# andreistana05/SAT-MPI-Stana-Andrei

Hardware: AMD Instinct MI355X
Metric: instances solved/sec, random 3-SAT n=100 α=4.26; unit-props/sec; HBM GB/s (higher is better)
Workload: dtype int32

## Files before the change

sat-mpi-stana-andrei_amd/csrc/dpll_scan.hip:

```cpp
#include <hip/hip_runtime.h>

#include <algorithm>
#include <climits>
#include <type_traits>

#include "common.h"
#include "dpll_scan.h"

#ifndef SATMI_SCAN_WAVES_PER_SIMD
#define SATMI_SCAN_WAVES_PER_SIMD 8
#endif

namespace satmi {
namespace {

#ifdef SATMI_PHASE_STAMPS
struct PhaseClock {
    uint64_t acc[8];
    uint64_t cnt[16];
    uint64_t t;
    __device__ void start() {
        for (int i = 0; i < 8; ++i) acc[i] = 0;
        for (int i = 0; i < 16; ++i) cnt[i] = 0;
        t = __builtin_amdgcn_s_memtime();
    }
    __device__ void count(int i, uint64_t v = 1) { cnt[i] += v; }
    __device__ void mark(int i) {
        const uint64_t x = __builtin_amdgcn_s_memtime();
        acc[i] += x - t;
        t = x;
    }
};
#else
struct PhaseClock {
    __device__ void start() {}
    __device__ void mark(int) {}
    __device__ void count(int, uint64_t = 1) {}
};
#endif
enum { PH_STAGE = 0, PH_ASSIGN = 1, PH_UNITS = 2, PH_CONFLICT = 3, PH_COUNTS = 4, PH_CHOOSE = 5, PH_PURE = 6,
       PH_OTHER = 7 };

constexpr uint32_t NONE32 = 0xFFFFFFFFu;


constexpr uint32_t LV_TRUE = 8u, LV_FALSE = 0u, LV_FREE = 1u;
constexpr uint32_t CODE_PAD = 0u, CODE_DUMMY = 1u;
__device__ __forceinline__ bool sum_true(uint32_t s) { return (s & 0xF8u) != 0u; }
__device__ __forceinline__ bool sum_open(uint32_t s) { return s < 8u; }
__device__ __forceinline__ uint32_t sum_nfree(uint32_t s) { return s & 7u; }

template <int K>
struct Pack;
template <>
struct Pack<3> {
    using W = uint32_t;
    static constexpr int BITS = 10;
    static constexpr int MAXV = 511;
    static constexpr int UNROLL = 7;
};
template <>
struct Pack<5> {
    using W = uint64_t;
    static constexpr int BITS = 12;
    static constexpr int MAXV = 2047;
    static constexpr int UNROLL = 2;
};

__host__ __device__ __forceinline__ int padded_clauses(int m) { return (m + 63) & ~63; }

template <int K>
__device__ __forceinline__ uint32_t field(typename Pack<K>::W w, int j) {
    return (uint32_t)(w >> (Pack<K>::BITS * j)) & ((1u << Pack<K>::BITS) - 1u);
}

struct ScanLayout {
    uint32_t cls, lv, ts, cnt, first, trail, fvar, ftrail, scratch, occ_off, bm, bytes;
    int32_t mcap, ncap, nw;
};

struct ScanArgs {
    const int32_t *inst_clause_begin, *clause_lit_begin, *lits, *inst_nvars;
    int32_t num_instances, sol_cap, sol_stride;
    int64_t max_solutions, node_limit;
    uint64_t time_limit_ticks;
    int32_t *status;
    int64_t *counters;
    int32_t *sol_len, *sol_lits, *root_len, *root_lits;
    uint32_t *work_counter;
    uint16_t *occ;
    int32_t occ_cap;
    ScanLayout lay;
    struct SplitCfg *split;
    int32_t occ_lists;
    uint32_t snap_lds;
};

template <int K, typename C>
struct SLds {
    static constexpr uint32_t PHASE_BIT = 1u << (8 * sizeof(C) - 1);
    typename Pack<K>::W *cls;
    uint8_t *lv;
    uint32_t *ts;
    uint32_t *cnt;
    uint32_t *first;
    C *trail;
    C *fvar;
    C *ftrail;
    C *snap;
    uint32_t *plist;
    C *snapg;
    uint32_t scap;
    uint16_t *occ_off;
    uint2 *bm;
    const uint16_t *occ;
};

__device__ __forceinline__ void lv_assign(uint8_t *lv, uint32_t code) {
    lv[code] = (uint8_t)LV_TRUE;
    lv[code ^ 1u] = (uint8_t)LV_FALSE;
}
__device__ __forceinline__ void lv_clear(uint8_t *lv, uint32_t v) {
    *(uint16_t *)(lv + 2 * v) = (uint16_t)(LV_FREE | (LV_FREE << 8));
}
__device__ __forceinline__ bool var_free(const uint8_t *lv, uint32_t v) { return (lv[2 * v] & 1u) != 0u; }

#include "dpll_scan_access.h"

template <int K, typename C>
constexpr bool plist_vars() { return sizeof(C) == 2 && K == 3; }
template <int K, typename C>
constexpr bool cnt_packed() {
#ifdef SATMI_CNT_PACK_ALL
    return K == 3;
#else
    return sizeof(C) == 2 && K == 3;
#endif
}
template <int K, typename C>
__device__ __forceinline__ void cnt_inc(const SLds<K, C> &S, uint32_t code, uint32_t inc) {
    if constexpr (!cnt_packed<K, C>()) atomicAdd(&S.cnt[code], inc);
    else atomicAdd(&S.cnt[code >> 1], inc << ((code & 1u) << 4));
}
template <int K, typename C>
__device__ __forceinline__ uint32_t cnt_fetch_inc(const SLds<K, C> &S, uint32_t code) {
    if constexpr (!cnt_packed<K, C>()) {
        return atomicAdd(&S.cnt[code], 1u);
    } else {
        const uint32_t sh = (code & 1u) << 4;
        return (atomicAdd(&S.cnt[code >> 1], 1u << sh) >> sh) & 0xFFFFu;
    }
}
template <int K, typename C>
__device__ __forceinline__ uint32_t cnt_get(const SLds<K, C> &S, uint32_t code) {
    if constexpr (!cnt_packed<K, C>()) return S.cnt[code];
    else return (S.cnt[code >> 1] >> ((code & 1u) << 4)) & 0xFFFFu;
}
template <int K, typename C>
__device__ __forceinline__ uint2 cnt_pair(const SLds<K, C> &S, uint32_t v) {
    if constexpr (!cnt_packed<K, C>()) {
        return ((const uint2 *)S.cnt)[v];
    } else {
        const uint32_t w = S.cnt[v];
        return make_uint2(w & 0xFFFFu, w >> 16);
    }
}
template <int K, typename C>
__device__ __forceinline__ void cnt_clear_var(const SLds<K, C> &S, uint32_t v) {
    if constexpr (!cnt_packed<K, C>()) ((uint2 *)S.cnt)[v] = make_uint2(0u, 0u);
    else S.cnt[v] = 0u;
}


template <int K, int U, typename C, typename F>
__device__ __forceinline__ void chunk_group(const SLds<K, C> &S, int c0, F &&f) {
    using W = typename Pack<K>::W;
// ... 21 lines not shown
    for (; c0 < mpad; c0 += 64) {
        const W w = S.cls[c0 + ln];
        uint32_t x[K];
#pragma unroll
        for (int j = 0; j < K; ++j) x[j] = lv_get(S, field<K>(w, j));
        f(c0 + ln, w, x);
    }
}

template <int K>
__device__ __forceinline__ uint32_t clause_sum(const uint32_t (&x)[K]) {
    uint32_t s = x[0];
#pragma unroll
    for (int j = 1; j < K; ++j) s += x[j];
    return s;
}

template <int K>
__device__ __forceinline__ uint32_t unit_code(typename Pack<K>::W w, const uint32_t (&x)[K]) {
    if constexpr (K == 3) {
        return __builtin_amdgcn_ubfe((uint32_t)w, x[1] * (uint32_t)Pack<3>::BITS + x[2] * (2u * Pack<3>::BITS),
                                     Pack<3>::BITS);
    } else {
        uint32_t code = field<K>(w, 0);
#pragma unroll
        for (int j = 1; j < K; ++j)
            if (x[j] & 1u) code = field<K>(w, j);
        return code;
    }
}

constexpr uint32_t EPOCH_LIMIT = 0xFFFFu - 4096u;
__device__ __forceinline__ uint32_t stamp(uint32_t ep, uint32_t k) { return ((ep << 16) | 0xFFFFu) - k; }
__device__ __forceinline__ uint32_t stamp_index(uint32_t st) { return 0xFFFFu - (st & 0xFFFFu); }

template <int K, typename C>
__device__ __forceinline__ void snap_put(const SLds<K, C> &S, uint32_t k, uint32_t code) {
    if constexpr (sizeof(C) == 1) {
        S.snap[k] = (C)code;
    } else {
        if (k < S.scap) S.snap[k] = (C)code;
        else S.snapg[k - S.scap] = (C)code;
    }
}
template <int K, typename C>
__device__ __forceinline__ uint32_t snap_get(const SLds<K, C> &S, uint32_t k) {
    if constexpr (sizeof(C) == 1) return S.snap[k];
    else return k < S.scap ? (uint32_t)S.snap[k] : (uint32_t)S.snapg[k - S.scap];
}
template <int K, typename C>
__device__ __forceinline__ void snap_ready(const SLds<K, C> &S, int nu) {
    if constexpr (sizeof(C) == 2)
        if ((uint32_t)nu > S.scap) __builtin_amdgcn_fence(__ATOMIC_SEQ_CST, "workgroup");
}

template <int K, typename C>
__device__ int scan_units(const SLds<K, C> &S, int mpad, uint32_t ep, uint32_t bep, int *empty_at) {
    using W = typename Pack<K>::W;
    const uint64_t lt = lanemask_lt();
    int nu = 0;
    int e = INT_MAX;
    for_chunks<K, Pack<K>::UNROLL>(S, mpad, [&](int c, W, const uint32_t(&x)[K]) {
        const uint32_t s = clause_sum<K>(x);
        const bool open = !sum_true(s);
        const uint32_t nf = sum_nfree(s);
        if (open && nf == 0u) {
            const W w = S.cls[c];
            int t = -1;
#pragma unroll
            for (int j = 0; j < K; ++j) {
                const uint32_t code = field<K>(w, j);
                const uint32_t st = code > CODE_DUMMY ? S.ts[code >> 1] : 0u;
                if ((st >> 16) == bep) t = max(t, (int)stamp_index(st));
            }
            e = min(e, t);
        }
        const bool unit = open && nf == 1u;
        const uint64_t mk = __ballot(unit);
        if (unit) {
            const uint32_t k = (uint32_t)nu + (uint32_t)__popcll(mk & lt);
            const uint32_t code = unit_code<K>(S.cls[c], x);
            snap_put(S, k, code);
            ts_stamp(S, code >> 1, stamp(ep, k));
        }
        nu += __popcll(mk);
    });
    wave_sync();
    *empty_at = __ballot(e != INT_MAX) ? wave_min_i32(e) : INT_MAX;
    return nu;
}

template <int K, typename C>
__device__ __forceinline__ int emptier(const SLds<K, C> &S, typename Pack<K>::W w, uint32_t bep) {
    int tt = -1;
#pragma unroll
    for (int j = 0; j < K; ++j) {
        const uint32_t code = field<K>(w, j);
        const uint32_t ts = S.ts[code >> 1];
        const uint32_t st = code > CODE_DUMMY ? ts : 0u;
        tt = (st >> 16) == bep ? max(tt, (int)stamp_index(st)) : tt;
    }
    return tt;
}

constexpr int FAST_UNITS = 2;
constexpr int FAST_BATCH = 16;

template <int K, typename C>
__device__ int inc_units(const SLds<K, C> &S, int nw, int rs, int tl, uint32_t ep, uint32_t bep, int *empty_at,
                         int *pre, PhaseClock &ph) {
    using W = typename Pack<K>::W;
    const int ln = lane_id();
    ph.count(0);
    ph.count(7, (uint64_t)(tl - rs));
    if (__builtin_expect(tl - rs <= FAST_BATCH, 1)) {
        const bool inb = ln < tl - rs;
        const uint32_t x = (uint32_t)S.trail[inb ? rs + ln : rs] ^ 1u;
        const int o0 = S.occ_off[x], o1 = S.occ_off[x + 1];
        const int ob = inb ? o0 : 0, len = inb ? o1 - o0 : 0;
        const int incl = row_incl_scan(len);
        const int excl = incl - len;
        const int delta = ob - excl;
        const int total = __builtin_amdgcn_readlane(incl, 15);
        if (__builtin_expect(total <= 64, 1)) {
            ph.count(1);
            int d = __builtin_amdgcn_readlane(delta, 0);
            if (tl - rs > 1)
            for (int b = 1; b < tl - rs; ++b) {
                const int eb = __builtin_amdgcn_readlane(excl, b);
                const int db = __builtin_amdgcn_readlane(delta, b);
                d = ln >= eb ? db : d;
            }
            const bool valid = ln < total;
            const uint32_t c = S.occ[(uint32_t)(valid ? d + ln : 0)];
            const W w = cls_at(S, c);
            uint32_t x[K];
#pragma unroll
            for (int j = 0; j < K; ++j) x[j] = lv_get(S, field<K>(w, j));
            const uint32_t sv = valid ? clause_sum<K>(x) : 0xFFu;
            const bool empty = sv == 0u;
            if (__builtin_expect(__ballot(empty) != 0ull, 0)) {
                ph.count(2);
                const int et = emptier<K>(S, w, bep);
                const int e = empty ? et : INT_MAX;
                *empty_at = wave_min_i32(e);
                return 0;
            }
            *empty_at = INT_MAX;
            const bool unit = sv == 1u;
            const uint64_t um = __ballot(unit);
            const int nun = __popcll(um);
            ph.count(4, (uint64_t)nun);
            ph.count(nun == 0 ? 10 : nun == 1 ? 11 : nun == 2 ? 12 : nun <= 8 ? 13 : 6, nun <= 8 ? 1 : 0);
            if (__builtin_expect(nun <= FAST_UNITS, 1)) {
                ph.count(3);
                uint64_t dm = um;
                int rank = 0;
                const uint32_t code = unit_code<K>(w, x);
                bool keep = unit;
                int nkeep = nun;
                if (nun == 2) {
                    const int u0 = __builtin_ctzll(um), u1 = 63 - __builtin_clzll(um);
                    const uint32_t c0 = (uint32_t)__builtin_amdgcn_readlane((int)c, u0);
                    const uint32_t c1 = (uint32_t)__builtin_amdgcn_readlane((int)c, u1);
                    const uint32_t v0 = (uint32_t)__builtin_amdgcn_readlane((int)code, u0) >> 1;
                    const uint32_t v1 = (uint32_t)__builtin_amdgcn_readlane((int)code, u1) >> 1;
                    dm = c0 == c1 ? 1ull << u0 : um;
                    rank = ln == u0 ? (c1 < c0 ? 1 : 0) : (c0 < c1 ? 1 : 0);
                    const bool one = (c0 == c1) | (v0 == v1);
                    keep = unit & (!one | (rank == 0));
                    nkeep = one ? 1 : 2;
                }
                if (keep) {
                    S.trail[tl + rank] = (C)code;
                    lv_assign(S.lv, code);
                    S.ts[code >> 1] = stamp(ep, (uint32_t)rank);
                }
                wave_sync();
                *pre = nkeep;
                return __popcll(dm);
            }
            if (unit) atomicOr(&S.bm[c >> 5].x, 1u << (c & 31u));
            wave_sync();
            int nu = 0;
            if (nw <= 64) {
                const uint32_t bits = ln < nw ? S.bm[ln].x : 0u;
                const int pc = __popc(bits);
                const int in = wave_incl_scan(pc);
                if (ln < nw) S.bm[ln].y = (uint32_t)(in - pc);
                nu = lane63(in);
            } else
            for (int w0 = 0; w0 < nw; w0 += 64) {
                const int wi = w0 + ln;
                const uint32_t bits = wi < nw ? S.bm[wi].x : 0u;
                const int pc = __popc(bits);
                const int in = wave_incl_scan(pc);
                if (wi < nw) S.bm[wi].y = (uint32_t)(nu + in - pc);
                nu += lane63(in);
            }
            wave_sync();
            if (unit) {
                const uint2 pb = S.bm[c >> 5];
                const uint32_t k = pb.y + (uint32_t)__popc(pb.x & ((1u << (c & 31u)) - 1u));
                const uint32_t code = unit_code<K>(w, x);
                snap_put(S, k, code);
                ts_stamp(S, code >> 1, stamp(ep, k));
                S.bm[c >> 5].x = 0u;
            }
            wave_sync();
            ph.count(6);
            return nu;
        }
    }
    ph.count(5);
    ph.count(tl - rs > FAST_BATCH ? 8 : 9);
    int e = INT_MAX;
    int passes = 0;
    bool unit = false;
    uint32_t uc = 0, ucode = 0;
    for (int i0 = rs; i0 < tl; i0 += 64) {
        const int i = i0 + ln;
        int ob = 0, len = 0;
        if (i < tl) {
            const uint32_t x = (uint32_t)S.trail[i] ^ 1u;
            ob = S.occ_off[x];
            len = (int)S.occ_off[x + 1] - ob;
        }
        const int incl = wave_incl_scan(len);
        const int excl = incl - len;
        const int delta = ob - excl;
        const int total = lane63(incl);
        const int nb = min(64, tl - i0);
        for (int t0 = 0; t0 < total; t0 += 64) {
            const int t = t0 + ln;
            int d = 0;
            for (int b = 0; b < nb; ++b) {
                const int eb = __builtin_amdgcn_readlane(excl, b);
                const int db = __builtin_amdgcn_readlane(delta, b);
                d = t >= eb ? db : d;
            }
            ++passes;
            if (t < total) {
                const uint32_t c = S.occ[d + t];
                const W w = cls_at(S, c);
                uint32_t x[K];
#pragma unroll
                for (int j = 0; j < K; ++j) x[j] = lv_get(S, field<K>(w, j));
                const uint32_t s = clause_sum<K>(x);
                if (!sum_true(s)) {
                    const uint32_t nf = sum_nfree(s);
                    if (nf == 0u) {
                        e = min(e, emptier<K>(S, w, bep));
                    } else if (nf == 1u) {
                        atomicOr(&S.bm[c >> 5].x, 1u << (c & 31u));
                        unit = true;
                        uc = c;
                        ucode = unit_code<K>(w, x);
                    }
                }
            }
        }
    }
    wave_sync();
    const int emp = __ballot(e != INT_MAX) ? wave_min_i32(e) : INT_MAX;
    *empty_at = emp;
    if (emp != INT_MAX) {
        for (int w = ln; w < nw; w += 64) S.bm[w].x = 0u;
        wave_sync();
        return 0;
    }
    int nu = 0;
    for (int w0 = 0; w0 < nw; w0 += 64) {
        const int w = w0 + ln;
        const uint32_t bits = w < nw ? S.bm[w].x : 0u;
        const int pc = __popc(bits);
        const int in = wave_incl_scan(pc);
        if (w < nw) S.bm[w].y = (uint32_t)(nu + in - pc);
        nu += lane63(in);
    }
    wave_sync();
    if (passes <= 1) {
        if (unit) {
            const uint2 p = S.bm[uc >> 5];
            const uint32_t k = p.y + (uint32_t)__popc(p.x & ((1u << (uc & 31u)) - 1u));
            snap_put(S, k, ucode);
            ts_stamp(S, ucode >> 1, stamp(ep, k));
        }
    } else {
        for (int w = ln; w < nw; w += 64) {
            const uint2 p = S.bm[w];
            uint32_t bits = p.x, k = p.y;
            while (bits) {
                const uint32_t c = ((uint32_t)w << 5) | (uint32_t)__builtin_ctz(bits);
                bits &= bits - 1u;
                const W wd = S.cls[c];
                uint32_t x[K];
#pragma unroll
                for (int j = 0; j < K; ++j) x[j] = lv_get(S, field<K>(wd, j));
                const uint32_t code = unit_code<K>(wd, x);
                snap_put(S, k, code);
                ts_stamp(S, code >> 1, stamp(ep, k));
                ++k;
            }
        }
    }
    wave_sync();
    for (int w = ln; w < nw; w += 64) S.bm[w].x = 0u;
    return nu;
}

template <int K, typename C>
__device__ uint32_t next_decision_epoch(const SLds<K, C> &S, int n, uint32_t ep) {
    if (ep < EPOCH_LIMIT) return ep + 1;
    for (int v = lane_id(); v <= n; v += 64) S.ts[v] = 0u;
    wave_sync();
    return 1;
}

template <int K, typename C>
__device__ __forceinline__ void assign_decision(const SLds<K, C> &S, int tl, uint32_t code, uint32_t ep) {
    S.trail[tl] = (C)code;
    lv_assign(S.lv, code);
    S.ts[code >> 1] = stamp(ep, 0u);
}

template <int K, bool INC, typename C>
__device__ bool propagate(const SLds<K, C> &S, int mpad, int &tl, int nu, bool dec, uint32_t &ep, uint32_t &props,
                          uint32_t &rounds, PhaseClock &ph) {
    const int ln = lane_id();
    int e = INT_MAX;
    int rs = tl;
    props -= dec ? 1u : 0u;
    ph.count(14);
// ... 133 lines not shown
    int npure = 0;
    uint32_t lmax = 0;
    auto count_step = [&](int v0) {
        const int v = v0 + ln;
        const uint32_t vc = (uint32_t)min(v, n);
        const bool live = (v <= n) & var_free(S.lv, vc);
        const uint2 c = cnt_pair(S, vc);
        const uint32_t p = c.x, q = c.y;
        lmax = live ? max(lmax, p + q) : lmax;
        npure += __popcll(__ballot(live & ((p + q) != 0u) & ((p == 0u) | (q == 0u))));
    };
    if constexpr (sizeof(C) == 1) {
        if (n >= 1) count_step(1);
        if (n >= 65) count_step(65);
    } else {
        for (int v0 = 1; v0 <= n; v0 += 64) count_step(v0);
    }
    const uint32_t maxc = wave_max_u32(lmax);
    int ncand = 0;
    uint32_t cvar = 0;
    auto flag_step = [&](int v0) {
        const int v = v0 + ln;
        const uint32_t vc = (uint32_t)min(v, n);
        const bool live = (v <= n) & var_free(S.lv, vc);
        const uint2 c = cnt_pair(S, vc);
        const uint32_t p = c.x, q = c.y;
        const bool pure = live & ((p + q) != 0u) & ((p == 0u) | (q == 0u));
        const bool cand = live & (p + q == maxc);
        const uint64_t cm = __ballot(cand);
        cvar = (ncand == 0 && cm) ? (uint32_t)v0 + (uint32_t)__builtin_ctzll(cm) : cvar;
        ncand += __popcll(cm);
        const uint32_t vw = v <= n ? vc : 0u;
        S.first[vw] = npure ? (pure ? NONE32 : 0u) : (cand ? 1u : 0u);
        cnt_clear_var(S, vw);
    };
    if constexpr (sizeof(C) == 1) {
        if (n >= 1) flag_step(1);
        if (n >= 65) flag_step(65);
    } else {
        for (int v0 = 1; v0 <= n; v0 += 64) flag_step(v0);
    }
    cnt_clear_var(S, 0u);
    S.first[0] = 0u;
    wave_sync();
    uint32_t best = 0;
    if (npure > 0) {
        first_of_pures<K>(S, mpad, npure);
        int k = 0;
        auto collect = [&](int v0) {
            const int v = v0 + ln;
            const uint32_t f = v <= n ? S.first[v] : 0u;
            const bool pure = f != 0u;
            const uint64_t mk = __ballot(pure);
            if constexpr (!plist_vars<K, C>()) {
                if (pure) S.plist[k + __popcll(mk & lt)] = f - 1u;
            } else {
                if (pure) ((C *)S.plist)[k + __popcll(mk & lt)] = (C)v;
            }
            k += __popcll(mk);
        };
        if constexpr (sizeof(C) == 1) {
            if (n >= 1) collect(1);
            if (n >= 65) collect(65);
        } else {
            for (int v0 = 1; v0 <= n; v0 += 64) collect(v0);
        }
        wave_sync();
    } else if (maxc > 0) {
        if (ncand == 1) {
            best = cvar;
        } else {
            const uint32_t bestf = first_flagged<K>(S, mpad);
            best = uniform_u32(field<K>(S.cls[bestf >> 3], (int)(bestf & 7u)) >> 1);
        }
    }
    return {npure, best};
}

template <int K, typename C>
__device__ int assign_pures(const SLds<K, C> &S, int npure, int tl) {
    const int ln = lane_id();
    const auto pos = [&](int j) -> uint32_t {
        if constexpr (!plist_vars<K, C>()) return S.plist[j];
        else return S.first[((const C *)S.plist)[j]] - 1u;
    };
    for (int i0 = 0; i0 < npure; i0 += 64) {
        const int i = i0 + ln;
        const uint32_t my = i < npure ? pos(i) : NONE32;
        int rank = 0;
        for (int j = 0; j < npure; ++j) rank += pos(j) < my ? 1 : 0;
        if (i < npure) {
            const uint32_t code = field<K>(S.cls[my >> 3], (int)(my & 7u));
            S.trail[tl + rank] = (C)code;
            lv_assign(S.lv, code);
        }
    }
    wave_sync();
    return tl + npure;
}

template <int K, typename C>
__device__ void store_assignment(const SLds<K, C> &S, int tl, int32_t *out) {
    for (int i = lane_id(); i < tl; i += 64) {
        const uint32_t code = S.trail[i];
        const int v = (int)(code >> 1);
        out[i] = (code & 1u) ? -v : v;
    }
}

enum { ST_PROPAGATE = 0, ST_ANALYZE = 1, ST_BACKTRACK = 2, ST_DONE = 3 };

template <int K, typename C>
__device__ void build_occurrences(const SLds<K, C> &S, uint16_t *occ, int m, int n) {
    using W = typename Pack<K>::W;
    const int ln = lane_id();
    auto each_slot = [&](auto &&f) {
        for (int c = ln; c < m; c += 64) {
            const W w = S.cls[c];
#pragma unroll
            for (int j = 0; j < K; ++j) {
                const uint32_t code = field<K>(w, j);
                bool dup = code <= CODE_DUMMY;
#pragma unroll
                for (int i = 0; i < j; ++i) dup |= field<K>(w, i) == code;
                if (!dup) f(c, code);
            }
        }
    };
    each_slot([&](int, uint32_t code) { cnt_inc(S, code, 1u); });
    wave_sync();
    int carry = 0;
    for (int x0 = 0; x0 < 2 * (n + 1); x0 += 64) {
        const int x = x0 + ln;
        const int cx = x < 2 * (n + 1) ? (int)cnt_get(S, (uint32_t)x) : 0;
        const int in = wave_incl_scan(cx);
        if (x < 2 * (n + 1)) {
            S.occ_off[x] = (uint16_t)(carry + in - cx);
            if constexpr (!cnt_packed<K, C>()) S.cnt[x] = 0u;
            else if (!(x & 1)) S.cnt[x >> 1] = 0u;
        }
        carry += lane63(in);
    }
    if (ln == 0) S.occ_off[2 * (n + 1)] = (uint16_t)carry;
    wave_sync();
    each_slot([&](int c, uint32_t code) {
        const uint32_t old = cnt_fetch_inc(S, code);
        occ[S.occ_off[code] + old] = (uint16_t)c;
    });
    wave_sync();
    if constexpr (!cnt_packed<K, C>())
        for (int x = ln; x < 2 * (n + 1); x += 64) S.cnt[x] = 0u;
    else
        for (int v = ln; v <= n; v += 64) S.cnt[v] = 0u;
    __builtin_amdgcn_fence(__ATOMIC_SEQ_CST, "workgroup");
    wave_sync();
}

struct Ctr32 {
    uint32_t nodes = 0, decisions = 0, props = 0, pures = 0, conflicts = 0, rounds = 0;
};
constexpr uint32_t FLUSH_NODES = 1u << 20;
constexpr uint32_t TIME_CHECK_NODES = 1024;

#define SATMI_RLX_AGENT __ATOMIC_RELAXED, __HIP_MEMORY_SCOPE_AGENT
template <typename T>
__device__ __forceinline__ T ld_agent(T *p) { return __hip_atomic_load(p, SATMI_RLX_AGENT); }
template <typename T>
__device__ __forceinline__ void st_agent(T *p, T v) { __hip_atomic_store(p, v, SATMI_RLX_AGENT); }
template <typename T>
__device__ __forceinline__ T add_agent(T *p, T v) { return __hip_atomic_fetch_add(p, v, SATMI_RLX_AGENT); }
template <typename T>
__device__ __forceinline__ T cas_agent(T *p, T expect, T v) {
    __hip_atomic_compare_exchange_strong(p, &expect, v, __ATOMIC_RELAXED, __ATOMIC_RELAXED, __HIP_MEMORY_SCOPE_AGENT);
    return expect;
}

__device__ uint64_t flush_counters(int64_t *ctr, Ctr32 &c, bool &flushed) {
    uint64_t total = 0;
    if (lane_id() == 0) {
        const uint32_t v[6] = {c.nodes, c.decisions, c.props, c.pures, c.conflicts, c.rounds};
        const int k[6] = {SATMI_CTR_NODES, SATMI_CTR_DECISIONS, SATMI_CTR_UNIT_PROPS, SATMI_CTR_PURE,
                          SATMI_CTR_CONFLICTS, SATMI_CTR_ROUNDS};
        if (!flushed) {
            for (int i = 0; i < 6; ++i) st_agent(&ctr[k[i]], (int64_t)v[i]);
            total = c.nodes;
        } else {
            total = (uint64_t)add_agent(&ctr[SATMI_CTR_NODES], (int64_t)c.nodes) + c.nodes;
            for (int i = 1; i < 6; ++i) add_agent(&ctr[k[i]], (int64_t)v[i]);
        }
    }
    flushed = true;
    c = Ctr32{};
    return (uint64_t)uniform_u32((uint32_t)total) | ((uint64_t)uniform_u32((uint32_t)(total >> 32)) << 32);
}

struct SplitCfg {
    uint32_t pub;
    uint32_t taken;
    uint32_t pad0[30];
    int32_t want;
    uint32_t pad1[31];
    uint32_t done;
    int32_t helpers;
    uint32_t claims, reclaims;
    unsigned long long handoffs;
    unsigned long long busy;
    uint32_t pad2[24];
    int32_t slot_cap, slot_bytes, dstack_cap;
    uint32_t epoch;
    int32_t max_helpers;
    uint32_t warm;
    int32_t cont_off;
    int32_t cont_fb;
    uint32_t pad3[24];
};
constexpr int SPLIT_POOL_OFF = 512;
static_assert(sizeof(SplitCfg) == SPLIT_POOL_OFF, "SplitCfg layout");
#ifndef SATMI_SPLIT_CHECK_NODES
#define SATMI_SPLIT_CHECK_NODES 64u
#endif
constexpr uint32_t SPLIT_CHECK_NODES = SATMI_SPLIT_CHECK_NODES;
constexpr int SPLIT_MAX_PER_WAVE = 8;
enum : uint32_t { SL_PENDING = 1, SL_RUNNING = 2, SL_DONE = 3, SL_RECLAIMED = 4, SL_HANDED = 5 };
struct SlotFlags {
    uint32_t state;
    uint32_t cancel;
};
struct SlotHdr {
    int32_t inst, tl0, dec_code, status, model_len;
    int32_t cont_task, cont_depth, cont_nd;
    int64_t ctr[SATMI_NCOUNTERS];
};
constexpr int SLOT_HDR_OFF = 128, SLOT_TRAIL_OFF = 256;
__host__ __device__ __forceinline__ int slot_frames_bytes(int ncap, int cb) { return ((ncap + 1) * cb + 127) & ~127; }
__host__ __device__ __forceinline__ int slot_cont_off(int ncap, int cb) {
    return SLOT_TRAIL_OFF + slot_frames_bytes(ncap, cb);
}
__host__ __device__ __forceinline__ int slot_bytes_for(int ncap, int cb) {
    return slot_cont_off(ncap, cb) + 2 * slot_frames_bytes(ncap, cb) + ((4 * (ncap + 1) + 127) & ~127);
}

struct SlotRef {
    SlotFlags *f;
    SlotHdr *h;
    uint32_t *trail;
};
__device__ __forceinline__ SlotRef slot_ref(const ScanArgs &A, int s) {
    unsigned char *p = (unsigned char *)A.split + SPLIT_POOL_OFF + (size_t)s * (size_t)A.split->slot_bytes;
    return {(SlotFlags *)p, (SlotHdr *)(p + SLOT_HDR_OFF), (uint32_t *)(p + SLOT_TRAIL_OFF)};
}
__device__ __forceinline__ uint32_t slot_state(const ScanArgs &A, uint32_t st) { return A.split->epoch << 4 | st; }
__device__ __forceinline__ int32_t *split_dstack(const SplitCfg *cfg, size_t w) {
    unsigned char *p = (unsigned char *)cfg + SPLIT_POOL_OFF + (size_t)cfg->slot_cap * (size_t)cfg->slot_bytes;
    return (int32_t *)p + w * (size_t)cfg->dstack_cap;
}

__device__ __forceinline__ void publish_state(uint32_t *flag, uint32_t v) {
    asm volatile("s_waitcnt vmcnt(0)" ::: "memory");
    if (lane_id() == 0) st_agent(flag, v);
}
__device__ __forceinline__ void acquire_agent() {
    __builtin_amdgcn_fence(__ATOMIC_ACQUIRE, "agent");
    asm volatile("s_waitcnt vmcnt(0)" ::: "memory");
}

__device__ __forceinline__ void put_words(uint32_t *dst, const void *lds, int nbytes) {
    const uint32_t *src = (const uint32_t *)lds;
    for (int i = lane_id_here(); 4 * i < nbytes; i += 64) st_agent(&dst[i], src[i]);
}

__device__ uint32_t next_event_after(const ScanArgs &A, uint64_t total) {
    uint64_t ev = A.time_limit_ticks ? TIME_CHECK_NODES : FLUSH_NODES;
    if (A.node_limit > 0) ev = min(ev, (uint64_t)A.node_limit + 1u - total);
    return (uint32_t)ev;
}

template <int K, typename C>
__device__ void try_donate(const ScanArgs &A, const SLds<K, C> &S, int depth, int b, int32_t *dst, int &nd) {
    constexpr uint32_t PHASE = SLds<K, C>::PHASE_BIT, DON = SLds<K, C>::PHASE_BIT;
    const int ln = lane_id_here();
    int old = 0;
    if (ln == 0) old = add_agent(&A.split->want, -1);
    if (uniform_i32(old) <= 0) {
        if (ln == 0) add_agent(&A.split->want, 1);
        return;
    }
    int j = -1;
    for (int d0 = 0; d0 < depth; d0 += 64) {
        const int d = d0 + ln;
        const bool open = d < depth && !((uint32_t)S.fvar[d] & PHASE) && !((uint32_t)S.ftrail[d] & DON);
        const uint64_t mk = __ballot(open);
        if (mk) {
            j = d0 + __builtin_ctzll(mk);
            break;
        }
    }
    int s = -1;
    if (j >= 0 && nd < A.split->dstack_cap) {
        uint32_t x = 0;
        if (ln == 0) x = add_agent(&A.split->pub, 1u);
        x = uniform_u32(x);
        if (x < (uint32_t)A.split->slot_cap) s = (int)x;
    }
    if (s < 0) {
        if (ln == 0) add_agent(&A.split->want, 1);
        return;
// ... 218 lines not shown
            bool leaf = false;
            Choice r{0, 0u};
            ph.mark(PH_OTHER);
            const int nact = scan_counts<K>(S, mpad);
            ph.mark(PH_COUNTS);
            if (nact == 0) {
                leaf = true;
            } else {
                r = choose<K>(S, n, mpad);
                if (r.npure == 0 && r.best_var == 0u) leaf = true;
            }
            ph.mark(PH_CHOOSE);
            if (!leaf && r.npure > 0) {
                tl = assign_pures<K>(S, r.npure, tl);
                ph.mark(PH_PURE);
                c.pures += (uint32_t)r.npure;
                ++c.nodes;
            } else if (!leaf) {
                const uint32_t v = r.best_var;
                ep = next_decision_epoch<K>(S, n, ep);
                if (ln == 0) {
                    S.fvar[depth] = (C)v;
                    S.ftrail[depth] = (C)tl;
                    assign_decision<K>(S, tl, v << 1, ep);
                }
                ++depth;
                ++c.decisions;
                ++c.nodes;
                nu = 1;
                dec_round = true;
                state = ST_PROPAGATE;
                wave_sync();
            } else {
                if (is_task) {
                    const SlotRef me = slot_ref(A, task);
                    put_words(me.trail, S.trail, tl * (int)sizeof(C));
                    if (lane_id_here() == 0) st_agent(&me.h->model_len, tl);
                } else if (sols < A.sol_cap) {
                    store_assignment<K>(S, tl, A.sol_lits + ((int64_t)b * A.sol_cap + sols) * A.sol_stride);
                    if (ln == 0) A.sol_len[(int64_t)b * A.sol_cap + sols] = tl;
                }
                ++sols;
                if (A.max_solutions > 0 && sols >= A.max_solutions) {
                    status = SATMI_DPLL_STOPPED;
                    state = ST_DONE;
                } else {
                    state = ST_BACKTRACK;
                }
            }
        }
        if (!SPLIT && state == ST_BACKTRACK) {
            state = ST_DONE;
            int top = depth - 1;
            while (top >= 0 && (uniform_u32(S.fvar[top]) & SLds<K, C>::PHASE_BIT)) --top;
            depth = top + 1;
            if (top >= 0) {
                const uint32_t fv = uniform_u32(S.fvar[top]);
                const int ft = (int)uniform_u32(S.ftrail[top]);
                for (int i = ft + lane_id_here(); i < tl; i += 64) lv_clear(S.lv, S.trail[i] >> 1);
                tl = ft;
                ep = next_decision_epoch<K>(S, n, ep);
                if (ln == 0) {
                    S.fvar[top] = (C)(fv | SLds<K, C>::PHASE_BIT);
                    assign_decision<K>(S, tl, (fv << 1) | 1u, ep);
                }
                ++c.decisions;
                ++c.nodes;
                nu = 1;
                dec_round = true;
                state = ST_PROPAGATE;
                wave_sync();
            }
        }
        if (SPLIT && state == ST_BACKTRACK) {
            state = ST_DONE;
            for (;;) {
                while (depth > 0 && (uniform_u32(S.fvar[depth - 1]) & SLds<K, C>::PHASE_BIT)) --depth;
                if (depth == 0) break;
                const int top = depth - 1;
                const uint32_t fv = uniform_u32(S.fvar[top]);
                const uint32_t ftw = uniform_u32(S.ftrail[top]);
                const int ft = (int)(ftw & ~DON);
                for (int i = ft + lane_id_here(); i < tl; i += 64) lv_clear(S.lv, S.trail[i] >> 1);
                tl = ft;
                wave_sync();
                if (ftw & DON) {
                    --nd;
                    const int s = uniform_i32(dst[nd]);
                    if (lane_id_here() == 0) S.ftrail[top] = (C)ft;
                    const int got = take_donation<K>(A, S, s, top, dst, nd, is_task ? task : -1, ctr, c, flushed,
                                                     t_start);
                    if (got == TAKE_HANDED) {
                        status = STATUS_HANDED;
                        break;
                    }
                    if (got == TAKE_CANCELLED) {
                        status = SATMI_DPLL_TIMEOUT;
                        break;
                    }
                    if (got != TAKE_LOCAL) {
                        const SlotRef r = slot_ref(A, s);
                        merge_counters(ctr, c, flushed, r.h);
                        if (got == TAKE_UNSAT) {
                            --depth;
                            continue;
                        }
                        deliver_model<C>(A, b, is_task ? task : -1, r.trail, uniform_i32(r.h->model_len));
                        sols = 1;
                        status = SATMI_DPLL_STOPPED;
                        break;
                    }
                }
                ep = next_decision_epoch<K>(S, n, ep);
                if (ln == 0) {
                    S.fvar[top] = (C)(fv | SLds<K, C>::PHASE_BIT);
                    assign_decision<K>(S, tl, (fv << 1) | 1u, ep);
                }
                ++c.decisions;
                ++c.nodes;
                nu = 1;
                dec_round = true;
                state = ST_PROPAGATE;
                wave_sync();
                break;
            }
        }
        if (__builtin_expect(c.nodes >= next_event, 0) && state != ST_DONE) {
            if (SPL) {
                if (is_task && uniform_u32(ld_agent(&slot_ref(A, task).f->cancel))) {
                    status = SATMI_DPLL_TIMEOUT;
                    state = ST_DONE;
                    continue;
                }
                if ((flushed || c.nodes >= SPL->warm) && uniform_i32(ld_agent(&SPL->want)) > 0)
                    try_donate<K>(A, S, depth, b, dst, nd);
            }
            if (!SPL || c.nodes >= next_flush) {
                const uint64_t total = flush_counters(ctr, c, flushed);
                if (A.node_limit > 0 && total > (uint64_t)A.node_limit) {
                    status = SATMI_DPLL_NODE_LIMIT;
                    state = ST_DONE;
                } else if (A.time_limit_ticks && __builtin_amdgcn_s_memrealtime() - t0 > A.time_limit_ticks) {
                    status = SATMI_DPLL_TIMEOUT;
                    state = ST_DONE;
                } else {
                    next_flush = next_event_after(A, total);
                }
            }
            next_event = SPL ? min(next_flush, c.nodes + SPLIT_CHECK_NODES) : next_flush;
        }
    }
#ifdef SATMI_PHASE_STAMPS
    ph.mark(PH_OTHER);
    if (!is_task && A.root_lits && A.sol_stride >= 48 && ln < 24)
        ((int64_t *)(A.root_lits + (int64_t)b * A.sol_stride))[ln] = (int64_t)(ln < 8 ? ph.acc[ln] : ph.cnt[ln - 8]);
#endif
    if (SPLIT && status == STATUS_HANDED) return false;
    if (SPLIT && nd > 0) cancel_donations(A, dst, nd);
    flush_counters(ctr, c, flushed);
    const int64_t ticks = (int64_t)(__builtin_amdgcn_s_memrealtime() - t_start);
    if (!is_task) {
        if (ln == 0) {
            A.status[b] = status;
            ctr[SATMI_CTR_SOLUTIONS] = sols;
            if (SPL) add_agent(&ctr[SATMI_CTR_TICKS], ticks);
            else ctr[SATMI_CTR_TICKS] = ticks;
        }
        return true;
    }
    if constexpr (SPLIT) {
        const SlotRef me = slot_ref(A, task);
        if (ln == 0) {
            st_agent(&me.h->status, status);
            st_agent(&ctr[SATMI_CTR_SOLUTIONS], sols);
            add_agent(&ctr[SATMI_CTR_TICKS], ticks);
        }
        asm volatile("s_waitcnt vmcnt(0)" ::: "memory");
        uint32_t prev = 0;
        if (ln == 0) prev = cas_agent(&me.f->state, slot_state(A, SL_RUNNING), slot_state(A, SL_DONE));
        if (uniform_u32(prev) != slot_state(A, SL_HANDED)) return false;
        acquire_agent();
        const int ctask = uniform_i32(me.h->cont_task), cdepth = uniform_i32(me.h->cont_depth);
        const int cnd = uniform_i32(me.h->cont_nd), tl0 = uniform_i32(me.h->tl0);
        int64_t *nctr = ctask >= 0 ? slot_ref(A, ctask).h->ctr : A.counters + (int64_t)b * SATMI_NCOUNTERS;
        if (ln == 0) {
            const int k[7] = {SATMI_CTR_NODES, SATMI_CTR_DECISIONS, SATMI_CTR_UNIT_PROPS, SATMI_CTR_PURE,
                              SATMI_CTR_CONFLICTS, SATMI_CTR_ROUNDS, SATMI_CTR_TICKS};
            for (int i = 0; i < 7; ++i) add_agent(&nctr[k[i]], ld_agent(&ctr[k[i]]));
        }
        uint32_t *cont = (uint32_t *)((unsigned char *)me.f + A.split->cont_off);
        const int fw = A.split->cont_fb / 4;
        for (int i = lane_id_here(); 4 * i < cdepth * (int)sizeof(C); i += 64) {
            ((uint32_t *)S.fvar)[i] = ld_agent(&cont[i]);
            ((uint32_t *)S.ftrail)[i] = ld_agent(&cont[fw + i]);
        }
        for (int i = lane_id_here(); i < cnd; i += 64) st_agent(&dst[i], (int32_t)ld_agent(&cont[2 * fw + i]));
        asm volatile("s_waitcnt vmcnt(0)" ::: "memory");
        acquire_agent();
        const int mine = status;
        task = ctask;
        is_task = ctask >= 0;
        ctr = nctr;
        flushed = true;
        depth = cdepth;
        nd = cnd;
        sols = 0;
        t_start = __builtin_amdgcn_s_memrealtime();
        next_flush = next_event_after(A, 0);
        next_event = min(next_flush, c.nodes + SPLIT_CHECK_NODES);
        if (mine == SATMI_DPLL_STOPPED) {
            deliver_model<C>(A, b, is_task ? task : -1, me.trail, uniform_i32(me.h->model_len));
            sols = 1;
            status = SATMI_DPLL_STOPPED;
            state = ST_DONE;
        } else if (mine != SATMI_DPLL_EXHAUSTED) {
            status = mine;
            state = ST_DONE;
        } else {
            for (int i = tl0 + lane_id_here(); i < tl; i += 64) lv_clear(S.lv, S.trail[i] >> 1);
            tl = tl0;
            status = SATMI_DPLL_EXHAUSTED;
            state = ST_BACKTRACK;
        }
        wave_sync();
        continue;
    }
    return false;
    }
}

__global__ void __launch_bounds__(64) split_init_kernel(SplitCfg *dst, SplitCfg cfg) {
    static_assert(sizeof(SplitCfg) % 4 == 0, "SplitCfg words");
    const uint32_t *src = (const uint32_t *)&cfg;
    for (int i = threadIdx.x; i < (int)(sizeof(SplitCfg) / 4); i += 64) ((uint32_t *)dst)[i] = src[i];
}

__device__ __forceinline__ int2 next_donation(SplitCfg *cfg, int num_instances) {
    const int ln = lane_id();
    for (uint32_t polls = 0;; ++polls) {
        if ((polls & 7u) == 0u && uniform_u32(ld_agent(&cfg->done)) >= (uint32_t)num_instances)
            return make_int2(-1, -1);
        const unsigned long long q = ld_agent((unsigned long long *)&cfg->pub);
        const uint32_t p = min(uniform_u32((uint32_t)q), (uint32_t)cfg->slot_cap);
        const uint32_t t = uniform_u32((uint32_t)(q >> 32));
        if (t >= p) {
            __builtin_amdgcn_s_sleep(127);
            continue;
        }
        uint32_t got = 0;
        if (ln == 0) got = cas_agent(&cfg->taken, t, t + 1u);
        if (uniform_u32(got) != t) continue;
        unsigned char *slot = (unsigned char *)cfg + SPLIT_POOL_OFF + (size_t)t * (size_t)cfg->slot_bytes;
        SlotFlags *f = (SlotFlags *)slot;
        const uint32_t pending = cfg->epoch << 4 | SL_PENDING;
        while ((uniform_u32(ld_agent(&f->state)) >> 4) != cfg->epoch) __builtin_amdgcn_s_sleep(2);
        uint32_t prev = 0;
        if (ln == 0) prev = cas_agent(&f->state, pending, (cfg->epoch << 4) | SL_RUNNING);
        if (uniform_u32(prev) != pending) {
            if (ln == 0) add_agent(&cfg->want, 1);
            continue;
        }
        if (ln == 0) add_agent(&cfg->claims, 1u);
        acquire_agent();
        return make_int2(uniform_i32(((SlotHdr *)(slot + SLOT_HDR_OFF))->inst), (int)t);
    }
}

template <int K, bool INC, typename C, bool SPLIT>
__device__ void run_queue(const ScanArgs &A, const SLds<K, C> &S, int32_t *dst) {
    SplitCfg *const SPL = SPLIT ? A.split : nullptr;
    const int ln = lane_id();
    bool draining = false;
    uint64_t busy = 0;
    for (;;) {
        int b = -1, task = -1;
        if (!draining) {
            uint32_t x = 0;
            if (ln == 0) x = atomicAdd(A.work_counter, 1u);
            x = uniform_u32(x);
            if (x < (uint32_t)A.num_instances) {
                b = (int)x;
            } else {
                if (!SPL) break;
                int h = 0;
                if (ln == 0) h = add_agent(&SPL->helpers, 1);
                if (uniform_i32(h) >= SPL->max_helpers) break;
                draining = true;
                if (ln == 0) add_agent(&SPL->want, 1);
            }
        }
        if (draining) {
            const int2 w = next_donation(SPL, A.num_instances);
            if (w.y < 0) break;
            b = w.x;
            task = w.y;
        }
        const uint64_t tb = SPLIT ? __builtin_amdgcn_s_memrealtime() : 0;
        const bool root_done = solve_instance<K, INC, C, SPLIT>(A, S, uniform_i32(b), uniform_i32(task), dst);
        if (SPLIT) busy += __builtin_amdgcn_s_memrealtime() - tb;
        if (SPL && ln == 0) {
            if (root_done) add_agent((int32_t *)&SPL->done, 1);
            if (draining) add_agent(&SPL->want, 1);
        }
        wave_sync();
    }
    if (SPL && ln == 0) add_agent(&SPL->busy, (unsigned long long)busy);
}
// ... 353 lines not shown
```

Baseline: 830,900.

## Add single-literal-list multi-unit fast path and sort occurrence lists

When a propagation round comes from a single trail literal and produces more units than the fast path handles, units are deduplicated with per-variable timestamps and a ballot-ranked trail write, replacing the bitmap-and-scan path. Occurrence lists are also insertion-sorted by clause index after they are built, so propagation visits clauses in order and trail order stays deterministic. Extra phase-stamp counters are added for profiling. The sort adds setup cost, and the timestamp dedup relies on ts_first picking a single winner per variable.

```diff
diff --git a/sat-mpi-stana-andrei_amd/csrc/dpll_scan.hip b/sat-mpi-stana-andrei_amd/csrc/dpll_scan.hip
--- a/sat-mpi-stana-andrei_amd/csrc/dpll_scan.hip
+++ b/sat-mpi-stana-andrei_amd/csrc/dpll_scan.hip
@@ -17,11 +17,11 @@
 #ifdef SATMI_PHASE_STAMPS
 struct PhaseClock {
     uint64_t acc[8];
-    uint64_t cnt[16];
+    uint64_t cnt[24];
     uint64_t t;
     __device__ void start() {
         for (int i = 0; i < 8; ++i) acc[i] = 0;
-        for (int i = 0; i < 16; ++i) cnt[i] = 0;
+        for (int i = 0; i < 24; ++i) cnt[i] = 0;
         t = __builtin_amdgcn_s_memtime();
     }
     __device__ void count(int i, uint64_t v = 1) { cnt[i] += v; }
@@ -349,6 +349,9 @@
             const int nun = __popcll(um);
             ph.count(4, (uint64_t)nun);
             ph.count(nun == 0 ? 10 : nun == 1 ? 11 : nun == 2 ? 12 : nun <= 8 ? 13 : 6, nun <= 8 ? 1 : 0);
+            if (nun > FAST_UNITS) ph.count(tl - rs == 1 ? 16 : tl - rs == 2 ? 17 : tl - rs <= 4 ? 18 : 19);
+            else if (nun == 2 && tl - rs == 1) ph.count(20);
+            const bool one_list = tl - rs == 1;
             if (__builtin_expect(nun <= FAST_UNITS, 1)) {
                 ph.count(3);
                 uint64_t dm = um;
@@ -376,6 +379,25 @@
                 wave_sync();
                 *pre = nkeep;
                 return __popcll(dm);
+            }
+            if (one_list) {
+                ph.count(21);
+                const uint32_t code = unit_code<K>(w, x);
+                const uint32_t v = unit ? code >> 1 : 0u;
+                const uint32_t st = stamp(ep, __builtin_amdgcn_mbcnt_hi((uint32_t)(um >> 32),
+                                                                        __builtin_amdgcn_mbcnt_lo((uint32_t)um, 0u)));
+                if (unit) ts_stamp(S, v, st);
+                wave_sync();
+                const bool first = unit & (ts_first(S, v) == st);
+                const uint64_t fm = __ballot(first);
+                if (first) {
+                    S.trail[__builtin_amdgcn_mbcnt_hi((uint32_t)(fm >> 32),
+                                                      __builtin_amdgcn_mbcnt_lo((uint32_t)fm, (uint32_t)tl))] = (C)code;
+                    lv_assign(S.lv, code);
+                }
+                wave_sync();
+                *pre = __popcll(fm);
+                return nun;
             }
             if (unit) atomicOr(&S.bm[c >> 5].x, 1u << (c & 31u));
             wave_sync();
@@ -815,6 +837,26 @@
         for (int x = ln; x < 2 * (n + 1); x += 64) S.cnt[x] = 0u;
     else
         for (int v = ln; v <= n; v += 64) S.cnt[v] = 0u;
+    __builtin_amdgcn_fence(__ATOMIC_SEQ_CST, "workgroup");
+    wave_sync();
+    for (int x = 2 + ln; x < 2 * (n + 1); x += 64) {
+        const int o0 = S.occ_off[x], o1 = S.occ_off[x + 1];
+        uint32_t last = o0 < o1 ? occ[o0] : 0u;
+        for (int i = o0 + 1; i < o1; ++i) {
+            const uint32_t key = occ[i];
+            if (key > last) {
+                last = key;
+                continue;
+            }
+            int j = i;
+            uint32_t prev = last;
+            do {
+                occ[j] = (uint16_t)prev;
+                --j;
+            } while (j > o0 && (prev = occ[j - 1]) > key);
+            occ[j] = (uint16_t)key;
+        }
+    }
     __builtin_amdgcn_fence(__ATOMIC_SEQ_CST, "workgroup");
     wave_sync();
 }
@@ -1339,7 +1381,7 @@
     }
 #ifdef SATMI_PHASE_STAMPS
     ph.mark(PH_OTHER);
-    if (!is_task && A.root_lits && A.sol_stride >= 48 && ln < 24)
+    if (!is_task && A.root_lits && A.sol_stride >= 48 && ln < (A.sol_stride >= 64 ? 32 : 24))
         ((int64_t *)(A.root_lits + (int64_t)b * A.sol_stride))[ln] = (int64_t)(ln < 8 ? ph.acc[ln] : ph.cnt[ln - 8]);
 #endif
     if (SPLIT && status == STATUS_HANDED) return false;
```

After: 840,800, median of 6. +1.2%, better.
